# Jisu-Linnea-Han/ClimateMachine.jl

Hardware: AMD Instinct MI355X
Metric: DG RHS DOF-updates/sec (higher is better)
Workload: dtype f64; 1 GPU; Held-Suarez dry GCM (BASELINE configs[2]), stacked cubed sphere 6x30x30x8 elements, N=4, LSRK54 explicit, hyperdiffusion (DryBiharmonic, horizontal), Rusanov, fp64; elements=43200, nodes_per_element=125, states=5, parallelism=element partition (Hilbert, whole columns), 1 rank(s), RCCL p2p halo

## Files before the change

### climatemachine.jl_amd/csrc/cmdg.hip

```cpp
#include <dlfcn.h>

#include <algorithm>
#include <new>
#include <tuple>

#include "rccl.h"
#include "stepping.h"

namespace cmdg {

namespace {
typedef int (*roctx_push_t)(const char *);
typedef int (*roctx_pop_t)();
roctx_push_t g_roctx_push = nullptr;
roctx_pop_t g_roctx_pop = nullptr;
int g_roctx_state = 0;
void roctx_resolve()
{
    g_roctx_state = -1;
    const char *names[] = {"librocprofiler-sdk-roctx.so.1", "librocprofiler-sdk-roctx.so", "libroctx64.so.4",
                           "libroctx64.so", nullptr};
    const char *want = getenv("CMDG_ROCTX");
    void *lib = nullptr;
    for (int i = 0; names[i] && !lib; ++i) lib = dlopen(names[i], RTLD_NOW | RTLD_NOLOAD);
// ... 114 lines not shown
    delete worker;
    worker = nullptr;
    if (s_comp) hipStreamSynchronize(s_comp);
    if (s_comm) hipStreamSynchronize(s_comm);
    prof_collect();
    if (graph_exec) hipGraphExecDestroy(graph_exec);
    if (nccl_comm && rccl::CommDestroy) rccl::CommDestroy(nccl_comm);
}

static __global__ void k_face_digest(const double *__restrict__ vgeo, int nvgeo,
                                     const double *__restrict__ sgeo,
                                     const int64_t *__restrict__ vmapM,
                                     const int64_t *__restrict__ vmapP,
                                     const int64_t *__restrict__ elemtobndy, int NQ, int NQV,
                                     int64_t nreal, int32_t *__restrict__ faceP,
                                     double *__restrict__ faceG, int *__restrict__ bad)
{
    const int Np = NQ * NQ * NQV, Nfph = NQ * NQV, Nfpv = NQ * NQ;
    const int Nfp = Nfph > Nfpv ? Nfph : Nfpv, NFT = 4 * Nfph + 2 * Nfpv;
    const int64_t I = (int64_t)blockIdx.x * blockDim.x + threadIdx.x;
    if (I >= nreal * NFT) return;
    const int64_t e = I / NFT;
    const int t = (int)(I % NFT);
    int f, n;
    if (t < 4 * Nfph) {
        f = t / Nfph;
        n = t % Nfph;
    } else {
        f = 4 + (t - 4 * Nfph) / Nfpv;
        n = (t - 4 * Nfph) % Nfpv;
    }
// ... 3 lines not shown
    switch (f) {
    case 0: vid = NQ * (a + NQ * b); break;
    case 1: vid = (NQ - 1) + NQ * (a + NQ * b); break;
    case 2: vid = a + NQ * NQ * b; break;
    case 3: vid = a + NQ * ((NQ - 1) + NQ * b); break;
    case 4: vid = n; break;
    default: vid = n + NQ * NQ * (NQV - 1); break;
    }
    int flags = 0;
    const int64_t idM = vmapM[o] - 1;
    if (idM != e * Np + vid) flags |= 1;
    int64_t idP = vmapP[o] - 1;
    if (elemtobndy[f + 6 * e] != 0) idP = e * Np + vid;
    if (idP < 0 || idP > 2147483647LL) flags |= 4;
    faceP[I] = (int32_t)idP;
    const double *sg = sgeo + 5 * o;
#pragma unroll
    for (int c = 0; c < 4; ++c) faceG[((int64_t)4 * e + c) * NFT + t] = sg[c];
    const double mi = vgeo[vid + (int64_t)Np * (VMI + (int64_t)nvgeo * e)];
    if (!(sg[SVMI] == mi)) flags |= 2;
    if (flags) atomicOr(bad, flags);
}

int EngineBase::init(const cmdg_desc *d)
{
    Np = NQ * NQ * NQV;
    Nfp = NQ * (NQ > NQV ? NQ : NQV);
    if (d->N[0] != d->N[1] || d->N[0] != NQ - 1 || d->N[2] != NQV - 1)
        return fail(CMDG_ERR_INVALID, "cmdg_create: polynomial orders do not match the engine");
    if (NQV != NQ && !d->Dv)
        return fail(CMDG_ERR_INVALID, "cmdg_create: Dv is required when the vertical order differs");
    nreal = d->nreal;
    nghost = d->nghost;
    nelem = nreal + nghost;
    nf_first = d->nf_first;
// ... 54 lines not shown
    HIPCHK(hipMemcpy(d_D, d->D, sizeof(double) * NQ * NQ, hipMemcpyHostToDevice));
    g.D = d_D;
    g.Dv = d_D;
    if (NQV != NQ) {
        HIPCHK(d_Dv.alloc(NQV * NQV));
        HIPCHK(hipMemcpy(d_Dv, d->Dv, sizeof(double) * NQV * NQV, hipMemcpyHostToDevice));
        g.Dv = d_Dv;
    }
    {
        const int NFT = 4 * NQ * NQV + 2 * NQ * NQ;
        const int64_t nt = std::max<int64_t>(nreal, 1) * NFT;
        DevBuf<int> d_bad;
        int bad = 0;
        HIPCHK(d_faceP.alloc(nt));
        HIPCHK(d_faceG.alloc(4 * nt));
        HIPCHK(d_bad.alloc_zeroed(1, s_comp));
        if (nreal > 0)
            hipLaunchKernelGGL(k_face_digest, dim3((unsigned)((nreal * NFT + 255) / 256)), dim3(256), 0,
                               s_comp, g.vgeo, g.nvgeo, g.sgeo, g.vmapM, g.vmapP, g.elemtobndy, NQ,
                               NQV, nreal, d_faceP.get(), d_faceG.get(), d_bad.get());
        hipError_t le = hipGetLastError();
        hipError_t ce = hipMemcpyAsync(&bad, d_bad, sizeof(int), hipMemcpyDeviceToHost, s_comp);
        hipError_t se = hipStreamSynchronize(s_comp);
        d_bad.reset();
        if (le != hipSuccess || ce != hipSuccess || se != hipSuccess)
            return fail(CMDG_ERR_HIP, "cmdg_create: digest of the face tables failed");
        if (bad & 1)
            return fail(CMDG_ERR_INVALID, "cmdg_create: vmapM is not the face numbering of Grids.jl:586-594");
        if (bad & 2)
            return fail(CMDG_ERR_INVALID, "cmdg_create: sgeo's vMI differs from vgeo's MI at the face nodes (Grids.jl:1097-1101)");
        if (bad & 4)
            return fail(CMDG_ERR_INVALID, "cmdg_create: too many elements for 32-bit face indices");
        g.faceP = d_faceP;
        g.faceG = d_faceG;
    }
    aux = d->state_auxiliary;
    const size_t nd = (size_t)Np * nelem;
    gf = gf_node_major() ? nullptr : d->state_gradient_flux;
    gf_user = gf_node_major() ? d->state_gradient_flux : nullptr;
    if (!gf) {
        HIPCHK(gf_own.alloc_zeroed(std::max<size_t>(nd * ngf, 1), s_comp));
        gf = gf_own;
    }
    hypgrad_user = ngl > 0 ? d->Qhypervisc_grad : nullptr;
    HIPCHK(hypgrad.alloc_zeroed(std::max<size_t>(nd * 3 * ngl, 1), s_comp));
    hypdiv = d->Qhypervisc_div;
    if (!hypdiv) {
        HIPCHK(hd_own.alloc_zeroed(std::max<size_t>(nd * nhyp, 1), s_comp));
        hypdiv = hd_own;
// ... 23 lines not shown
{
    for (int i = 0; i < 2; ++i)
        if (!W[i]) {
            const size_t n = (size_t)Np * ns * nelem;
            HIPCHK(W[i].alloc_zeroed(n, s_comp));
            HIPCHK(hipStreamSynchronize(s_comp));
        }
    return CMDG_OK;
}

int EngineBase::ensure_garg()
{
    if (!garg) {
        const size_t n = std::max<size_t>((size_t)Np * ngl * nelem, 1);
        HIPCHK(garg.alloc_zeroed(n, s_comp));
        HIPCHK(hipStreamSynchronize(s_comp));
    }
    return CMDG_OK;
}

int EngineBase::synchronize()
{
    HIPCHK(hipStreamSynchronize(s_comp));
    HIPCHK(hipStreamSynchronize(s_comm));
    return CMDG_OK;
}

ProfRec &EngineBase::prof_pair(int kernel, bool clamp, Event e1)
{
    ProfRec r{kernel, Event(), std::move(e1), clamp};
// ... 663 lines not shown
```

### climatemachine.jl_amd/csrc/cmdg_common.h

```cpp
#pragma once
#include <hip/hip_runtime.h>
#include <stdint.h>

namespace cmdg {

enum { XI1X1 = 0, XI2X1, XI3X1, XI1X2, XI2X2, XI3X2, XI1X3, XI2X3, XI3X3, VM, VMI };
constexpr int JCV = 15;
enum { SN1 = 0, SN2, SN3, SSM, SVMI };
enum { DIR_EVERY = 0, DIR_HORIZONTAL = 1, DIR_VERTICAL = 2 };
enum {
    NF_RUSANOV = 0, NF_CENTRAL = 1, NF_ROE = 2, NF_HLLC = 3, NF_LMARS = 4,
    NF_ROE_MOIST = 5, NF_ROE_MOIST_LM = 6, NF_ROE_MOIST_HH = 7, NF_ROE_MOIST_LV = 8,
    NF_ROE_MOIST_LVPP = 9
};
enum { BS_FIRST = 0, BS_GRADIENT = 1 };

constexpr int NXCD = 8;

struct GridDev {
    const double *vgeo, *sgeo;
    const int64_t *vmapM, *vmapP, *elemtobndy;
    const double *D;
    const double *Dv;
    int nvgeo;
    const int32_t *faceP;
    const double *faceG;
};

struct SendEnt {
    int32_t node;
    int32_t pos;
};
struct HaloDev {
    const int32_t *sendoff;
    const SendEnt *sendent;
    double *send[2];
    const int32_t *ghostslot;
    const double *recvQ, *recvGF, *recvHG, *recvHD;
    int64_t nreal;
};

// ... 9 lines not shown
    __device__ __forceinline__ static void face_task(int t, int &f, int &n)
    {
        if constexpr (NQ == NQV) {
            f = t / Nfp;
            n = t % Nfp;
        } else if (t < 4 * Nfph) {
            f = t / Nfph;
            n = t % Nfph;
        } else {
            f = 4 + (t - 4 * Nfph) / Nfpv;
            n = (t - 4 * Nfph) % Nfpv;
        }
    }
};

__device__ __forceinline__ int64_t xcd_remap(int64_t b, int64_t G)
{
    const int64_t q = G / NXCD, r = G % NXCD;
    const int64_t x = b % NXCD, y = b / NXCD;
    return x * q + (x < r ? x : r) + y;
}

template <int N>
__device__ __forceinline__ void fill_negzero(double (&a)[N])
{
#pragma unroll
    for (int i = 0; i < N; ++i) a[i] = -0.0;
}
template <int N>
struct Vec {
// ... 55 lines not shown
    } else {
#pragma unroll
        for (int s = 0; s < NLOAD; ++s) dst[s] = arr[hg_at<NHG, Np>(vidP, s, eP)];
    }
}
template <int NHG, int Np, int NW>
__device__ __forceinline__ void store_node_major(double *__restrict__ arr, int64_t e, int tid, int nthreads,
                                                 const double *src)
{
    double *dst = arr + (int64_t)NHG * Np * e;
    for (int m = tid; m < NHG * Np; m += nthreads) {
        const int n = m / NHG, s = m - n * NHG;
        if (NW == NHG || s < NW) dst[m] = src[s * Np + n];
    }
}
template <int NVAR, int NW, class F>
__device__ __forceinline__ void send_nodes(const HaloDev &h, int which, int64_t e, int tid,
                                           int nthreads, F value)
{
    if (h.sendoff == nullptr || h.send[which] == nullptr) return;
    const int b1 = h.sendoff[e + 1];
    for (int k = h.sendoff[e] + tid; k < b1; k += nthreads) {
        const SendEnt ent = h.sendent[k];
        double *dst = h.send[which] + (int64_t)NVAR * ent.pos;
#pragma unroll
        for (int s = 0; s < NW; ++s) dst[s] = value(s, ent.node);
    }
}

}
// ... 1 lines not shown
```

### climatemachine.jl_amd/csrc/engine.h

```cpp
#pragma once
#include "engine_base.h"
#include "kernels.h"

namespace cmdg {

template <class P, int NQ_, int NQV_ = NQ_>
struct EngineT : EngineBase {
    typename P::Params prm;
    PassArgs<P> make_args(const RhsCtx &c, const int64_t *elems, int64_t n, int dir, bool exterior, double *send0,
                          double *send1) const
    {
        PassArgs<P> a;
        a.prm = prm;
        a.g = g;
        a.elems = elems;
        a.nelems = n;
        a.Q = c.Qin;
        a.aux = aux;
        a.aux_rw = aux;
        a.derived = derived;
        a.gf = gf;
        a.hypgrad = hypgrad;
        a.hypdiv = hypdiv;
        a.tendency = c.tendency;
        a.Qout = c.Qout;
        a.garg = garg;
        a.t = c.t;
        a.tptr = c.tptr;
        a.alpha = c.alpha;
        a.beta = c.beta;
        a.rkb_dt = c.rkb_dt;
        a.rka_next = c.rka_next;
        a.direction = dir;
        a.model_dir = direction;
        a.nf_first = nf_first;
        a.h = halo_dev(exterior, send0, send1);
        return a;
    }
    using Kernel = void (*)(PassArgs<P>);
    static constexpr bool HO = GradArgHandoff<P, NQ_, NQV_>::value;
    static constexpr bool ELIDE = GradArgHandoff<P, NQ_, NQV_>::elide_refresh;
// ... 24 lines not shown
    static Kernel tendency_recv(bool recv)
    {
        return recv ? k_tendency<P, NQ_, NQV_, LSRK, GF, true> : k_tendency<P, NQ_, NQV_, LSRK, GF, false>;
    }
    static Kernel pick_tendency(bool lsrk, bool gf, bool recv, GargOut out)
    {
        if constexpr (HO)
            if (out != GargOut::none) {
                if constexpr (ELIDE)
                    if (out == GargOut::records) return k_tendency<P, NQ_, NQV_, true, false, false, true, false>;
                return k_tendency<P, NQ_, NQV_, true, false, false, true>;
            }
        if (lsrk) return gf ? tendency_recv<true, true>(recv) : tendency_recv<true, false>(recv);
        return gf ? tendency_recv<false, true>(recv) : tendency_recv<false, false>(recv);
    }
    void launch_gradients(const RhsCtx &c, const int64_t *elems, int64_t n, bool exterior, hipStream_t st) override
    {
        in_pass(GRADIENTS, n, exterior, st, [&] {
            const PassArgs<P> args = make_args(c, elems, n, diffusion_direction, exterior,
                                               gf_live() ? slot[SLOT_GF].sendbuf : nullptr,
                                               ngl > 0 ? slot[SLOT_HG].sendbuf : nullptr);
            hipLaunchKernelGGL(pick_gradients(gf_live(), c.garg_in), dim3((unsigned)n), dim3(KDims<NQ_, NQV_>::NT), 0,
                               st, args);
        });
    }
    void launch_divgrad(const RhsCtx &c, const int64_t *elems, int64_t n, bool exterior, hipStream_t st) override
    {
        in_pass(DIVGRAD, n, exterior, st, [&] {
            const PassArgs<P> args = make_args(c, elems, n, diffusion_direction, exterior, slot[SLOT_HD].sendbuf, nullptr);
            hipLaunchKernelGGL((k_divgrad<P, NQ_, NQV_>), dim3((unsigned)n), dim3(KDims<NQ_, NQV_>::NT), 0, st, args);
        });
    }
    void launch_gradlap(const RhsCtx &c, const int64_t *elems, int64_t n, bool exterior, hipStream_t st) override
    {
        in_pass(GRADLAP, n, exterior, st, [&] {
            const PassArgs<P> args = make_args(c, elems, n, diffusion_direction, exterior, slot[SLOT_HG].sendbuf, nullptr);
            hipLaunchKernelGGL((k_gradlap<P, NQ_, NQV_>), dim3((unsigned)n), dim3(KDims<NQ_, NQV_>::NT), 0, st, args);
        });
    }
    void launch_tendency(const RhsCtx &c, const int64_t *elems, int64_t n, bool exterior, hipStream_t st) override
    {
        in_pass(TENDENCY, n, exterior, st, [&] {
            using SH = TendencyShape<P, NQ_, NQV_>;
            PassArgs<P> args = make_args(c, elems, n, direction, exterior, c.lsrk ? slot[SLOT_Q].sendbuf : nullptr, nullptr);
            const bool recv = args.h.ghostslot != nullptr && exterior;
            if (!recv) args.h.ghostslot = nullptr;
            hipLaunchKernelGGL(pick_tendency(c.lsrk, P::needs_gradflux(prm), recv, c.garg_out),
                               dim3((unsigned)SH::blocks(n)), dim3(SH::NT), 0, st, args);
        });
    }
    void launch_update_aux(const RhsCtx &c, int64_t e0, int64_t e1) override
    {
// ... 68 lines not shown
```

### climatemachine.jl_amd/csrc/engine_base.h

```cpp
#pragma once
#include <hip/hip_runtime.h>
#include <stdint.h>

#include <algorithm>
#include <condition_variable>
#include <deque>
#include <functional>
#include <mutex>
#include <optional>
#include <string>
#include <thread>
#include <vector>

#include "../../include/cmdg.h"
#include "cmdg_common.h"
#include "owned.h"

namespace cmdg {

enum { SLOT_Q = 0, SLOT_GF = 1, SLOT_HG = 2, SLOT_HD = 3, NSLOT = 4 };
enum { TRANSPORT_NONE = 0, TRANSPORT_LOCAL = 1, TRANSPORT_RCCL = 2 };

struct HaloSlot {
    DevBuf<double> sendbuf, recvbuf;
// ... 9 lines not shown
struct StepInRun {
    bool first_step, last_step;
};

enum class GargOut { none, records, records_refresh };

struct RhsCtx {
    double *tendency = nullptr;
    double *Qin = nullptr;
    double *Qout = nullptr;
    double t = 0, alpha = 1, beta = 0;
    const double *tptr = nullptr;
    bool lsrk = false;
    bool update_after = false;
    bool garg_in = false;
    GargOut garg_out = GargOut::none;
    double rkb_dt = 0, rka_next = 0;
    bool pre_done = false;
};

struct FilterObj {
    int kind = 0, target = 0, direction = 0;
    int nindices = 0;
    int indices[CMDG_MAX_FILTER_STATES] = {0};
    int aux_ref_rho = 0, aux_ref_rhoe = 0;
    DevBuf<double> d_Fh, d_Fv;
};

void roctx_push(const char *name);
void roctx_pop();
// ... 83 lines not shown
    int64_t nreal = 0, nghost = 0, nelem = 0;
    int ns = 0, naux = 0, ngrad = 0, ngf = 0, ngl = 0, nhyp = 0;
    int nf_first = 0, direction = 0, diffusion_direction = 0, stacked = 0;
    GridDev g{};
    const int64_t *d_interior = nullptr, *d_exterior = nullptr;
    const int64_t *d_interior_user = nullptr, *d_exterior_user = nullptr;
    DevBuf<int64_t> d_interior_tiled, d_exterior_tiled;
    int set_stack_height(int nv);
    int set_stream_priority(int level);
    int stream_priority = 0;
    int64_t ninterior = 0, nexterior = 0;
    const uint8_t *d_activedofs = nullptr;
    DevBuf<double> d_D;
    DevBuf<int32_t> d_faceP;
    DevBuf<double> d_faceG;
    const int64_t *d_vmapsend = nullptr, *d_vmaprecv = nullptr;
    int64_t nvmapsend = 0, nvmaprecv = 0;
    std::vector<int> nabrtorank;
    std::vector<int64_t> nabrsend, nabrrecv;
    double *aux = nullptr, *gf = nullptr, *hypdiv = nullptr;
    DevBuf<double> hypgrad;
    DevBuf<double> derived;
    DevBuf<double> gf_own, hd_own;
    double *hypgrad_user = nullptr, *gf_user = nullptr;
    DevBuf<double> gf_scratch;
    bool node_major(const double *array) const
    {
        return array == hypgrad || (array == gf && gf_node_major());
    }
    int dev = 0;
    Event ev_comp;
    HaloSlot slot[NSLOT];
    int slot_nvar_max = 0;
    DevBuf<double> W[2];
    DevBuf<double> garg;
    bool gradarg_handoff = true;
    bool handoff_used = false;
    int64_t handoff_refreshes = 0;
    virtual bool garg_capable() const = 0;
    virtual bool refresh_elidable() const = 0;
    bool handoff_eligible() const
    {
        return gradarg_handoff && garg_capable() && !gf_live() && ngl > 0 && has_update_aux() &&
               fused_update_aux() && !has_hooks && !step_filter && !tendency_filter && !gradient_filter &&
               !step_graph && nghost == 0 && !communicate();
    }
    int ensure_garg();
    DevBuf<double> d_partial;
    int transport = TRANSPORT_NONE;
    int rank = 0, nranks = 1;
// ... 245 lines not shown
```

### climatemachine.jl_amd/csrc/kernels.h

```cpp
#pragma once
#include <type_traits>

#include "cmdg_common.h"

#ifndef CMDG_TEND_MINW
#define CMDG_TEND_MINW 1
#endif
#ifndef CMDG_TEND_EPB_LARGE
#define CMDG_TEND_EPB_LARGE 2
#endif
#ifndef CMDG_TEND_EPB_SMALL
#define CMDG_TEND_EPB_SMALL 1
#endif
#ifndef CMDG_GRAD_MINW
#define CMDG_GRAD_MINW 4
#endif
#ifndef CMDG_GRAD_BOUND_LARGE
#define CMDG_GRAD_BOUND_LARGE 1024
#endif
#ifndef CMDG_LAP_MINW
#define CMDG_LAP_MINW 1
#endif

namespace cmdg {
// ... 2 lines not shown
struct PassArgs {
    typename P::Params prm;
    GridDev g;
    const int64_t *elems;
    int64_t nelems;
    const double *Q;
    const double *aux;
    double *aux_rw;
    const double *derived;
    double *gf;
    double *hypgrad;
    double *hypdiv;
    double *tendency;
    double *Qout;
    double *garg;
    double t, alpha, beta;
    const double *tptr;
    double rkb_dt, rka_next;
    int direction;
    int model_dir;
    int nf_first;
    HaloDev h;
};

struct FacePt {
    double n[3], sM, vMI;
    int64_t eP;
    int vidM, vidP, bctag;
};

template <int NQ, int NQV = NQ>
__host__ __device__ __forceinline__ constexpr int face_vid(int f, int n)
{
    const int a = n % NQ, b = n / NQ;
    switch (f) {
    case 0: return NQ * (a + NQ * b);
    case 1: return (NQ - 1) + NQ * (a + NQ * b);
    case 2: return a + NQ * NQ * b;
    case 3: return a + NQ * ((NQ - 1) + NQ * b);
    case 4: return n;
    default: return n + NQ * NQ * (NQV - 1);
    }
}

template <int NQ, int NQV = NQ>
__device__ __forceinline__ void face_index(const GridDev &g, int64_t e, int t, int f, int32_t &idP,
                                           int &bctag)
{
    idP = g.faceP[(int64_t)KDims<NQ, NQV>::NFT * e + t];
    bctag = (int)g.elemtobndy[f + 6 * e];
}
template <int NQ, int NQV = NQ>
__device__ __forceinline__ void face_geometry(const GridDev &g, int64_t e, int t, int f, int n,
                                              int32_t idP, int bctag, FacePt &fp)
{
    constexpr int Np = KDims<NQ, NQV>::Np, NFT = KDims<NQ, NQV>::NFT;
    const double *sg = g.faceG + (int64_t)4 * NFT * e + t;
    fp.n[0] = sg[0];
    fp.n[1] = sg[NFT];
    fp.n[2] = sg[2 * NFT];
    fp.sM = sg[3 * NFT];
    fp.vidM = face_vid<NQ, NQV>(f, n);
    fp.vMI = g.vgeo[fp.vidM + (int64_t)Np * (VMI + (int64_t)g.nvgeo * e)];
    fp.bctag = bctag;
    fp.eP = idP / Np;
    fp.vidP = idP - (int)fp.eP * Np;
}
template <int NQ, int NQV = NQ>
__device__ __forceinline__ void face_setup(const GridDev &g, int64_t e, int t, int f, int n,
                                           FacePt &fp)
{
    int32_t idP;
    int bctag;
    face_index<NQ, NQV>(g, e, t, f, idP, bctag);
    face_geometry<NQ, NQV>(g, e, t, f, n, idP, bctag, fp);
}

template <class P, class = void>
struct has_flux_wavespeed : std::false_type {
};
template <class P>
struct has_flux_wavespeed<P, std::void_t<decltype(P::HAS_FLUX_WAVESPEED)>> : std::true_type {
};

template <class P, class = void>
struct gf_node_major : std::false_type {
};
template <class P>
struct gf_node_major<P, std::void_t<decltype(P::GF_NODE_MAJOR)>>
    : std::integral_constant<bool, P::GF_NODE_MAJOR && (P::NGF > 0)> {
// ... 651 lines not shown
            if (vt) law_gradient_flux<P>(a.prm, o2, gv, lQ, laux, a_t, Gn);
#pragma unroll
            for (int s = 0; s < NGF; ++s)
                sA[s * Np + tid] = hz ? (vt ? o1[s] + o2[s] : o1[s]) : o2[s];
        }
    }
    __syncthreads();
    Vec<NACC> corr;
    int vidM = 0, fpair = -1;
    if (tid < KD::NFT) {
        int f, n;
        KD::face_task(tid, f, n);
        const bool on = f < 4 ? hz : vt;
        if (on) {
            FacePt fp;
            face_setup<NQ, NQV>(a.g, e, tid, f, n, fp);
            Vec<NS> QM, QP;
            Vec<NAUX> auxM, auxP;
            Vec<NGRAD> GM, GP;
            if constexpr (!GARG_IN) {
                load_state<NS, Np>(QM, a.Q, fp.vidM, e);
                load_state<NAUX, Np>(auxM, a.aux, fp.vidM, e);
            }
#pragma unroll
            for (int s = 0; s < NGRAD; ++s)
                GM[s] = (GMASK >> s & 1) ? sG[s * Np + fp.vidM] : 0.0;
            GP.negzero();
            Vec<NGF> lgf;
            lgf.negzero();
            Vec<3 * NGRAD> tg, nGM;
            if (fp.bctag == 0) {
// ... 34 lines not shown
#pragma unroll
                for (int s = 0; s < NGRAD; ++s)
#pragma unroll
                    for (int d = 0; d < 3; ++d) tg[d + 3 * s] = fp.n[d] * GP[s];
            }
            if constexpr (NGF > 0) law_gradient_flux<P>(a.prm, lgf, tg, QM, auxM, a_t, GM);
#pragma unroll
            for (int s = 0; s < NGRAD; ++s)
#pragma unroll
                for (int d = 0; d < 3; ++d) nGM[d + 3 * s] = fp.n[d] * GM[s];
#pragma unroll
            for (int s = 0; s < NGL; ++s)
#pragma unroll
                for (int d = 0; d < 3; ++d) {
                    const int q = d + 3 * P::hv_indexmap(s);
                    corr[NGF + 3 * s + d] = fp.vMI * fp.sM * (tg[q] - nGM[q]);
                }
            if constexpr (NGF > 0) {
                Vec<NGF> visc;
                for (int s = 0; s < NGF; ++s) visc[s] = 0;
                law_gradient_flux<P>(a.prm, visc, nGM, QM, auxM, a_t, GM);
#pragma unroll
                for (int s = 0; s < NGF; ++s) corr[s] = fp.vMI * fp.sM * (lgf[s] - visc[s]);
            }
            vidM = fp.vidM;
            fpair = f / 2;
        }
    }
#pragma unroll
    for (int p = 0; p < 3; ++p) {
        if (fpair == p) {
#pragma unroll
            for (int s = 0; s < NACC; ++s) sA[s * Np + vidM] += corr[s];
        }
        __syncthreads();
    }
    if (tid < Np) {
        if constexpr (!gf_node_major<P>::value) {
// ... 1 lines not shown
            for (int s = 0; s < NGF; ++s)
                a.gf[tid + (int64_t)Np * (s + (int64_t)P::NGF * e)] = sA[s * Np + tid];
        }
    }
    if constexpr (gf_node_major<P>::value && NGF > 0)
        store_node_major<P::NGF, Np, NGF>(a.gf, e, tid, (int)blockDim.x, sA);
    if constexpr (NHG > 0)
        store_node_major<NHG, Np, NHG>(a.hypgrad, e, tid, (int)blockDim.x, sA + NGF * Np);
    if constexpr (NGF > 0)
        send_nodes<P::NGF, NGF>(a.h, 0, e, tid, (int)blockDim.x, [&](int s, int n) { return sA[s * Np + n]; });
    if constexpr (NHG > 0)
        send_nodes<NHG, NHG>(a.h, 1, e, tid, (int)blockDim.x,
                             [&](int s, int n) { return sA[(NGF + s) * Np + n]; });
}

template <class P, int NQ, int NQV = NQ>
__global__ void __launch_bounds__((KDims<NQ, NQV>::NT)) k_divgrad(const PassArgs<P> a)
{
    using KD = KDims<NQ, NQV>;
    const double a_t = a.tptr ? *a.tptr : a.t;
    constexpr int Np = KD::Np, NAUX = P::NAUX, NGL = P::NGL, NHG = 3 * NGL,
                  NHYP = P::NHYP, NG = NGL > 0 ? NGL : 1;
    __shared__ double sD[NQ * NQ + (NQV == NQ ? 0 : NQV * NQV)];
    const double *const sDv = sD + (NQV == NQ ? 0 : NQ * NQ);
    __shared__ double sC[3 * NG * Np];
    __shared__ double sA[NG * Np];
    constexpr int NSURF = SurfDims<NQ, NQV>::NSURF;
    __shared__ double sM[(NHG > 0 ? NHG : 1) * NSURF];
    const int tid = threadIdx.x;
    const int64_t e = a.elems[xcd_remap(blockIdx.x, gridDim.x)] - 1;
    if (tid < NQ * NQ) sD[tid] = a.g.D[tid];
// ... 49 lines not shown
                for (int kk = 0; kk < NQV; ++kk)
                    dv -= MI * sDv[kk + NQV * k] * sC[(2 * NG + s) * Np + i + NQ * (j + NQ * kk)];
            }
            sA[s * Np + tid] = hz ? (vt ? dh + dv : dh) : dv;
        }
    }
    __syncthreads();
    Vec<NGL> corr;
    int vidM = 0, fpair = -1;
    if (tid < KD::NFT) {
        int f, n;
        KD::face_task(tid, f, n);
        const bool on = f < 4 ? hz : vt;
        if (on) {
            FacePt fp;
            face_setup<NQ, NQV>(a.g, e, tid, f, n, fp);
            Vec<NHG> gM, gP;
            const int sidx = surf_index<NQ, NQV>(fp.vidM);
#pragma unroll
            for (int q = 0; q < NHG; ++q) gM[q] = sM[q * NSURF + sidx];
            load_plus_hg<NHG, Np, NHG>(gP, a.hypgrad, a.h.recvHG, ghost_slot<Np>(a.h, fp.eP, fp.vidP),
                                    fp.vidP, fp.eP);
            if (fp.bctag != 0) {
                Vec<NAUX> auxM, auxP;
                load_state<NAUX, Np>(auxM, a.aux, fp.vidM, e);
                load_state<NAUX, Np>(auxP, a.aux, fp.vidP, fp.eP);
                P::boundary_state_divergence(a.prm, fp.bctag, gP, auxP, fp.n, gM, auxM, a_t);
            }
            const double nh0 = fp.n[0] / 2, nh1 = fp.n[1] / 2, nh2 = fp.n[2] / 2;
#pragma unroll
            for (int s = 0; s < NGL; ++s) {
                const double ldiv = (gP[3 * s] + gM[3 * s]) * nh0 +
                                    (gP[3 * s + 1] + gM[3 * s + 1]) * nh1 +
                                    (gP[3 * s + 2] + gM[3 * s + 2]) * nh2;
                corr[s] = fp.vMI * fp.sM * ldiv;
            }
            vidM = fp.vidM;
            fpair = f / 2;
        }
    }
#pragma unroll
    for (int p = 0; p < 3; ++p) {
        if (fpair == p) {
#pragma unroll
            for (int s = 0; s < NGL; ++s) sA[s * Np + vidM] += corr[s];
        }
        __syncthreads();
    }
    if (tid < Np) {
#pragma unroll
        for (int s = 0; s < NGL; ++s)
            a.hypdiv[tid + (int64_t)Np * (s + (int64_t)NHYP * e)] = sA[s * Np + tid];
    }
    if constexpr (NGL > 0)
        send_nodes<NGL, NGL>(a.h, 0, e, tid, (int)blockDim.x, [&](int s, int n) { return sA[s * Np + n]; });
}

template <class P, int NQ, int NQV = NQ>
__global__ void __launch_bounds__((KDims<NQ, NQV>::NT), CMDG_LAP_MINW) k_gradlap(const PassArgs<P> a)
{
    using KD = KDims<NQ, NQV>;
    const double a_t = a.tptr ? *a.tptr : a.t;
    constexpr int Np = KD::Np, NS = P::NS, NAUX = P::NAUX, NGL = P::NGL,
                  NHG = 3 * NGL, NHYP = P::NHYP, NG = NGL > 0 ? NGL : 1,
                  NH = NHYP > 0 ? NHYP : 1;
    __shared__ double sD[NQ * NQ + (NQV == NQ ? 0 : NQV * NQV)];
    const double *const sDv = sD + (NQV == NQ ? 0 : NQ * NQ);
    __shared__ double sL[NG * Np];
    __shared__ double sA[NH * Np];
    const int tid = threadIdx.x;
    const int64_t e = a.elems[xcd_remap(blockIdx.x, gridDim.x)] - 1;
    if (tid < NQ * NQ) sD[tid] = a.g.D[tid];
    if constexpr (NQV != NQ) {
        if (tid < NQV * NQV) sD[NQ * NQ + tid] = a.g.Dv[tid];
    }
    const bool hz = a.direction != DIR_VERTICAL, vt = a.direction != DIR_HORIZONTAL;
    if (tid < Np) {
        Vec<NGL> l;
#pragma unroll
        for (int s = 0; s < NGL; ++s) l[s] = a.hypdiv[tid + (int64_t)Np * (s + (int64_t)NHYP * e)];
#pragma unroll
        for (int s = 0; s < NGL; ++s) sL[s * Np + tid] = l[s];
    }
    __syncthreads();
    if (tid < Np) {
        const int i = tid % NQ, j = (tid / NQ) % NQ, k = tid / (NQ * NQ);
        const double *vg = a.g.vgeo + (int64_t)Np * a.g.nvgeo * e + tid;
        Vec<NS> lQ;
        Vec<NAUX> laux;
        load_state<NS, Np>(lQ, a.Q, tid, e);
        load_state<NAUX, Np>(laux, a.aux, tid, e);
        Vec<NHG> lh, lv;
        lh.negzero();
        lv.negzero();
        if (hz) {
// ... 33 lines not shown
        h2.negzero();
        if (hz) P::post_gradient_laplacian(a.prm, h1, lh, lQ, laux, a_t);
        if (vt) P::post_gradient_laplacian(a.prm, h2, lv, lQ, laux, a_t);
#pragma unroll
        for (int s = 0; s < NHYP; ++s) sA[s * Np + tid] = hz ? (vt ? h1[s] + h2[s] : h1[s]) : h2[s];
    }
    __syncthreads();
    Vec<NHYP> corr;
    int vidM = 0, fpair = -1;
    if (tid < KD::NFT) {
        int f, n;
        KD::face_task(tid, f, n);
        const bool on = f < 4 ? hz : vt;
        if (on) {
            FacePt fp;
            face_setup<NQ, NQV>(a.g, e, tid, f, n, fp);
            Vec<NS> QM, QP;
            Vec<NAUX> auxM, auxP;
            Vec<NGL> lapM, lapP;
            load_state<NS, Np>(QM, a.Q, fp.vidM, e);
            load_state<NAUX, Np>(auxM, a.aux, fp.vidM, e);
            const int gslot = ghost_slot<Np>(a.h, fp.eP, fp.vidP);
            load_plus<NS, Np, NS>(QP, a.Q, a.h.recvQ, gslot, fp.vidP, fp.eP);
            load_state<NAUX, Np>(auxP, a.aux, fp.vidP, fp.eP);
#pragma unroll
            for (int s = 0; s < NGL; ++s) lapM[s] = sL[s * Np + fp.vidM];
            load_plus<NHYP, Np, NGL, NGL>(lapP, a.hypdiv, a.h.recvHD, gslot, fp.vidP, fp.eP);
            if (fp.bctag != 0)
                P::boundary_state_higher_order(a.prm, fp.bctag, QP, auxP, lapP, fp.n, QM, auxM,
                                               lapM, a_t);
            Vec<NHG> G;
#pragma unroll
            for (int s = 0; s < NGL; ++s)
#pragma unroll
                for (int d = 0; d < 3; ++d) G[d + 3 * s] = fp.n[d] * (lapP[s] - lapM[s]) / 2;
            Vec<NHYP> lh;
            for (int s = 0; s < NHYP; ++s) lh[s] = 0;
            P::post_gradient_laplacian(a.prm, lh, G, QM, auxM, a_t);
#pragma unroll
            for (int s = 0; s < NHYP; ++s) corr[s] = fp.vMI * fp.sM * lh[s];
            vidM = fp.vidM;
            fpair = f / 2;
        }
    }
#pragma unroll
    for (int p = 0; p < 3; ++p) {
        if (fpair == p) {
#pragma unroll
            for (int s = 0; s < NHYP; ++s) sA[s * Np + vidM] += corr[s];
        }
        __syncthreads();
    }
    if constexpr (NHYP > 0) store_node_major<NHG, Np, NHYP>(a.hypgrad, e, tid, (int)blockDim.x, sA);
    if constexpr (NHYP > 0)
        send_nodes<NHG, NHYP>(a.h, 0, e, tid, (int)blockDim.x, [&](int s, int n) { return sA[s * Np + n]; });
// ... 100 lines not shown
```

### climatemachine.jl_amd/csrc/lsrk_run.hip

```cpp
#include "stepping.h"

namespace cmdg {

static __global__ void k_lsrk_update(double *__restrict__ dQ, double *__restrict__ Q, double rka,
                                     double rkb_dt, int64_t n)
{
    for (int64_t i = blockIdx.x * (int64_t)blockDim.x + threadIdx.x; i < n;
         i += (int64_t)gridDim.x * blockDim.x) {
        Q[i] += rkb_dt * dQ[i];
        dQ[i] *= rka;
    }
}
void lsrk_update(hipStream_t st, double *dQ, double *Q, double rka_next, double rkb_dt, int64_t n)
{
    hipLaunchKernelGGL(k_lsrk_update, dim3(nblocks(n)), dim3(256), 0, st, dQ, Q, rka_next, rkb_dt, n);
}
void lsrk_update(EngineBase *e, double *dQ, double *Q, double rka_next, double rkb_dt)
{
    lsrk_update(e->s_comp, dQ, Q, rka_next, rkb_dt, real_len(e));
}

static void lsrk_stage_buffers(EngineBase *e, double *Q, int s, int nstages, double **in, double **out)
{
    *in = s == 0 ? Q : e->W[(s - 1) % 2];
    *out = s == nstages - 1 && nstages > 1 ? Q : e->W[s % 2];
}

struct StageHandoff {
    bool garg_in;
    GargOut out;
};
static StageHandoff handoff_stage(const StepInRun *run, int s, int nstages, bool refresh_elidable)
{
    if (!run) return {false, GargOut::none};
    const bool in = !(run->first_step && s == 0);
    if (run->last_step && s == nstages - 1) return {in, GargOut::none};
    const bool refresh = !refresh_elidable || nstages == 1 || (run->last_step && s == nstages - 2);
    return {in, refresh ? GargOut::records_refresh : GargOut::records};
}

int EngineBase::lsrk_step(double *Q, double *dQ, double t, double dt, int nstages, const double *rka,
                          const double *rkb, const double *rkc, bool continued, const StepInRun *handoff)
{
    std::vector<EngineBase *> one{this};
    double *Qs[1] = {Q}, *dQs[1] = {dQ};
    if (transport == TRANSPORT_LOCAL && communicate())
        return fail(CMDG_ERR_INVALID, "handles connected locally must be driven by the cmdg_group_* calls");
    return group_lsrk_step(one, Qs, dQs, t, dt, nstages, rka, rkb, rkc, continued, nullptr, handoff);
}

int group_lsrk_step(std::vector<EngineBase *> &g, double **Q, double **dQ, double t, double dt,
                    int nstages, const double *rka, const double *rkb, const double *rkc,
                    bool continued, const double *stage_times_dev, const StepInRun *handoff)
// ... 12 lines not shown
                x.Qin = Q[i];
                x.Qout = nullptr;
            }
            x.tendency = dQ[i];
            x.t = t + rkc[s] * dt;
            x.tptr = stage_times_dev ? stage_times_dev + s : nullptr;
            x.alpha = 1.0;
            x.beta = 1.0;
            x.lsrk = fused;
            x.update_after = !fused;
            x.rkb_dt = rkb[s] * dt;
            x.rka_next = rka[(s + 1) % nstages];
            const StageHandoff h = handoff_stage(handoff, s, nstages, g[i]->refresh_elidable());
            x.garg_in = h.garg_in;
            x.garg_out = h.out;
            if (h.out == GargOut::records_refresh) g[i]->handoff_refreshes += 1;
        }
        if (int r = group_rhs(g, c, s > 0 || continued)) return r;
    }
    for (size_t i = 0; i < g.size(); ++i) {
        EngineBase *e = g[i];
        if (nstages == 1 && e->fused_lsrk())
            if (hipMemcpyAsync(Q[i], e->W[0], sizeof(double) * e->Np * e->ns * e->nreal,
                               hipMemcpyDeviceToDevice, e->s_comp) != hipSuccess)
                return e->fail(CMDG_ERR_HIP, "lsrk: copy back failed");
        if (e->step_filter) {
            if (int r = e->filter_apply(e->step_filter, Q[i], e->ns)) return r;
            e->invalidate_sends();
        }
    }
// ... 195 lines not shown
```

Before: 19.11 billion DOF-updates/s.

## Store Laplacian in ring-major records and precompute face lift weights

Face digest now precomputes a per-face-point lift weight (vMI*sM) and a ring-slot-remapped neighbour index. In the handoff path, divgrad writes its Laplacian output to a new ring-major buffer and skips the hypdiv store except on the final evaluation. gradlap then reads neighbour Laplacian values from that buffer via the remapped index and skips loading the plus-side state and aux, reusing the minus side instead. This cuts scattered global loads and extra geometry fetches in the hyperdiffusion face loops, at the cost of two more face tables and another Laplacian buffer. It also assumes the plus-side state and aux are not needed in this path, which holds only if the boundary and flux laws never use them.

```diff
diff --git a/climatemachine.jl_amd/csrc/cmdg.hip b/climatemachine.jl_amd/csrc/cmdg.hip
--- a/climatemachine.jl_amd/csrc/cmdg.hip
+++ b/climatemachine.jl_amd/csrc/cmdg.hip
@@ -152,7 +152,8 @@
                                      const int64_t *__restrict__ vmapP,
                                      const int64_t *__restrict__ elemtobndy, int NQ, int NQV,
                                      int64_t nreal, int32_t *__restrict__ faceP,
-                                     double *__restrict__ faceG, int *__restrict__ bad)
+                                     double *__restrict__ faceG, double *__restrict__ faceW,
+                                     int32_t *__restrict__ facePr, int *__restrict__ bad)
 {
     const int Np = NQ * NQ * NQV, Nfph = NQ * NQV, Nfpv = NQ * NQ;
     const int Nfp = Nfph > Nfpv ? Nfph : Nfpv, NFT = 4 * Nfph + 2 * Nfpv;
@@ -186,11 +187,14 @@
     if (elemtobndy[f + 6 * e] != 0) idP = e * Np + vid;
     if (idP < 0 || idP > 2147483647LL) flags |= 4;
     faceP[I] = (int32_t)idP;
+    const int64_t eP = idP >= 0 ? idP / Np : 0;
+    facePr[I] = (int32_t)(eP * Np + ring_slot_of(NQ, NQV, (int)(idP - eP * Np)));
     const double *sg = sgeo + 5 * o;
 #pragma unroll
     for (int c = 0; c < 4; ++c) faceG[((int64_t)4 * e + c) * NFT + t] = sg[c];
     const double mi = vgeo[vid + (int64_t)Np * (VMI + (int64_t)nvgeo * e)];
     if (!(sg[SVMI] == mi)) flags |= 2;
+    faceW[I] = mi * sg[SSM];
     if (flags) atomicOr(bad, flags);
 }
 
@@ -275,11 +279,14 @@
         int bad = 0;
         HIPCHK(d_faceP.alloc(nt));
         HIPCHK(d_faceG.alloc(4 * nt));
+        HIPCHK(d_faceW.alloc(nt));
+        HIPCHK(d_facePr.alloc(nt));
         HIPCHK(d_bad.alloc_zeroed(1, s_comp));
         if (nreal > 0)
             hipLaunchKernelGGL(k_face_digest, dim3((unsigned)((nreal * NFT + 255) / 256)), dim3(256), 0,
                                s_comp, g.vgeo, g.nvgeo, g.sgeo, g.vmapM, g.vmapP, g.elemtobndy, NQ,
-                               NQV, nreal, d_faceP.get(), d_faceG.get(), d_bad.get());
+                               NQV, nreal, d_faceP.get(), d_faceG.get(), d_faceW.get(), d_facePr.get(),
+                               d_bad.get());
         hipError_t le = hipGetLastError();
         hipError_t ce = hipMemcpyAsync(&bad, d_bad, sizeof(int), hipMemcpyDeviceToHost, s_comp);
         hipError_t se = hipStreamSynchronize(s_comp);
@@ -294,6 +301,8 @@
             return fail(CMDG_ERR_INVALID, "cmdg_create: too many elements for 32-bit face indices");
         g.faceP = d_faceP;
         g.faceG = d_faceG;
+        g.faceW = d_faceW;
+        g.facePr = d_facePr;
     }
     aux = d->state_auxiliary;
     const size_t nd = (size_t)Np * nelem;
@@ -347,6 +356,7 @@
     if (!garg) {
         const size_t n = std::max<size_t>((size_t)Np * ngl * nelem, 1);
         HIPCHK(garg.alloc_zeroed(n, s_comp));
+        HIPCHK(lapr.alloc_zeroed(n, s_comp));
         HIPCHK(hipStreamSynchronize(s_comp));
     }
     return CMDG_OK;
diff --git a/climatemachine.jl_amd/csrc/cmdg_common.h b/climatemachine.jl_amd/csrc/cmdg_common.h
--- a/climatemachine.jl_amd/csrc/cmdg_common.h
+++ b/climatemachine.jl_amd/csrc/cmdg_common.h
@@ -25,6 +25,8 @@
     int nvgeo;
     const int32_t *faceP;
     const double *faceG;
+    const double *faceW;
+    const int32_t *facePr;
 };
 
 struct SendEnt {
@@ -64,6 +66,68 @@
     }
 };
 
+__host__ __device__ __forceinline__ constexpr int ring_slot_of(int NQ, int NQV, int n)
+{
+    const int i = n % NQ, j = (n / NQ) % NQ, k = n / (NQ * NQ), E = NQ - 1;
+    const int c = j == 0 ? i
+                  : i == E ? E + j
+                  : j == E ? 2 * E + (E - i)
+                  : i == 0 ? 3 * E + (E - j)
+                           : 4 * E + (i - 1) + (NQ - 2) * (j - 1);
+    return c * NQV + k;
+}
+__host__ __device__ __forceinline__ constexpr int ring_node_of(int NQ, int NQV, int slot)
+{
+    const int c = slot / NQV, k = slot - c * NQV, E = NQ - 1, NI = NQ > 2 ? NQ - 2 : 1;
+    const int q = c - 4 * E;
+    const int i = c <= E ? c : c <= 2 * E ? E : c <= 3 * E ? 3 * E - c : c < 4 * E ? 0 : 1 + q % NI;
+    const int j = c <= E ? 0 : c <= 2 * E ? c - E : c <= 3 * E ? E : c < 4 * E ? 4 * E - c : 1 + q / NI;
+    return i + NQ * (j + NQ * k);
+}
+template <int NQ, int NQV = NQ>
+__host__ __device__ __forceinline__ constexpr int ring_slot(int n)
+{
+    return ring_slot_of(NQ, NQV, n);
+}
+template <int NQ, int NQV = NQ>
+__host__ __device__ __forceinline__ constexpr int ring_node(int slot)
+{
+    return ring_node_of(NQ, NQV, slot);
+}
+template <int NQ, int NQV>
+constexpr bool ring_order_ok()
+{
+    constexpr int Np = NQ * NQ * NQV, R = 4 * (NQ - 1) * NQV, Nfph = NQ * NQV;
+    for (int n = 0; n < Np; ++n) {
+        const int s = ring_slot<NQ, NQV>(n);
+        if (s < 0 || s >= Np || ring_node<NQ, NQV>(s) != n) return false;
+    }
+    for (int s = 0; s < Np; ++s)
+        if (ring_slot<NQ, NQV>(ring_node<NQ, NQV>(s)) != s) return false;
+    for (int f = 0; f < 4; ++f) {
+        bool on[R] = {};
+        int count = 0;
+        for (int n = 0; n < Np; ++n) {
+            const int i = n % NQ, j = (n / NQ) % NQ;
+            if (f == 0 ? i == 0 : f == 1 ? i == NQ - 1 : f == 2 ? j == 0 : j == NQ - 1) {
+                const int s = ring_slot<NQ, NQV>(n);
+                if (s >= R || on[s]) return false;
+                on[s] = true;
+                ++count;
+            }
+        }
+        if (count != Nfph) return false;
+        int starts = 0;
+        for (int s = 0; s < R; ++s)
+            if (on[s] && !on[(s + R - 1) % R]) ++starts;
+        if (starts != 1) return false;
+    }
+    return true;
+}
+static_assert(ring_order_ok<3, 3>() && ring_order_ok<4, 4>() && ring_order_ok<5, 5>(), "ring order");
+static_assert(ring_order_ok<2, 2>() && ring_order_ok<6, 6>() && ring_order_ok<7, 7>(), "ring order");
+static_assert(ring_order_ok<5, 3>() && ring_order_ok<3, 5>() && ring_order_ok<5, 2>(), "ring order");
+
 __device__ __forceinline__ int64_t xcd_remap(int64_t b, int64_t G)
 {
     const int64_t q = G / NXCD, r = G % NXCD;
@@ -149,6 +213,17 @@
         if (NW == NHG || s < NW) dst[m] = src[s * Np + n];
     }
 }
+template <int NHG, int NQ, int NQV>
+__device__ __forceinline__ void store_ring_major(double *__restrict__ arr, int64_t e, int tid, int nthreads,
+                                                 const double *src)
+{
+    constexpr int Np = KDims<NQ, NQV>::Np;
+    double *dst = arr + (int64_t)NHG * Np * e;
+    for (int m = tid; m < NHG * Np; m += nthreads) {
+        const int r = m / NHG, s = m - r * NHG;
+        dst[m] = src[s * Np + ring_node<NQ, NQV>(r)];
+    }
+}
 template <int NVAR, int NW, class F>
 __device__ __forceinline__ void send_nodes(const HaloDev &h, int which, int64_t e, int tid,
                                            int nthreads, F value)
diff --git a/climatemachine.jl_amd/csrc/engine.h b/climatemachine.jl_amd/csrc/engine.h
--- a/climatemachine.jl_amd/csrc/engine.h
+++ b/climatemachine.jl_amd/csrc/engine.h
@@ -25,6 +25,8 @@
         a.tendency = c.tendency;
         a.Qout = c.Qout;
         a.garg = garg;
+        a.lapr = lapr;
+        a.hypdiv_out = c.hypdiv_out;
         a.t = c.t;
         a.tptr = c.tptr;
         a.alpha = c.alpha;
@@ -79,6 +81,18 @@
         if (lsrk) return gf ? tendency_recv<true, true>(recv) : tendency_recv<true, false>(recv);
         return gf ? tendency_recv<false, true>(recv) : tendency_recv<false, false>(recv);
     }
+    static Kernel pick_divgrad(bool ring)
+    {
+        if constexpr (HO)
+            if (ring) return k_divgrad<P, NQ_, NQV_, true>;
+        return k_divgrad<P, NQ_, NQV_>;
+    }
+    static Kernel pick_gradlap(bool ring)
+    {
+        if constexpr (HO)
+            if (ring) return k_gradlap<P, NQ_, NQV_, true>;
+        return k_gradlap<P, NQ_, NQV_>;
+    }
     void launch_gradients(const RhsCtx &c, const int64_t *elems, int64_t n, bool exterior, hipStream_t st) override
     {
         in_pass(GRADIENTS, n, exterior, st, [&] {
@@ -93,14 +107,15 @@
     {
         in_pass(DIVGRAD, n, exterior, st, [&] {
             const PassArgs<P> args = make_args(c, elems, n, diffusion_direction, exterior, slot[SLOT_HD].sendbuf, nullptr);
-            hipLaunchKernelGGL((k_divgrad<P, NQ_, NQV_>), dim3((unsigned)n), dim3(KDims<NQ_, NQV_>::NT), 0, st, args);
+            hipLaunchKernelGGL(pick_divgrad(c.garg_in), dim3((unsigned)n), dim3(KDims<NQ_, NQV_>::NT), 0, st, args);
         });
     }
     void launch_gradlap(const RhsCtx &c, const int64_t *elems, int64_t n, bool exterior, hipStream_t st) override
     {
         in_pass(GRADLAP, n, exterior, st, [&] {
-            const PassArgs<P> args = make_args(c, elems, n, diffusion_direction, exterior, slot[SLOT_HG].sendbuf, nullptr);
-            hipLaunchKernelGGL((k_gradlap<P, NQ_, NQV_>), dim3((unsigned)n), dim3(KDims<NQ_, NQV_>::NT), 0, st, args);
+            PassArgs<P> args = make_args(c, elems, n, diffusion_direction, exterior, slot[SLOT_HG].sendbuf, nullptr);
+            if (c.garg_in) args.g.faceP = g.facePr;
+            hipLaunchKernelGGL(pick_gradlap(c.garg_in), dim3((unsigned)n), dim3(KDims<NQ_, NQV_>::NT), 0, st, args);
         });
     }
     void launch_tendency(const RhsCtx &c, const int64_t *elems, int64_t n, bool exterior, hipStream_t st) override
diff --git a/climatemachine.jl_amd/csrc/engine_base.h b/climatemachine.jl_amd/csrc/engine_base.h
--- a/climatemachine.jl_amd/csrc/engine_base.h
+++ b/climatemachine.jl_amd/csrc/engine_base.h
@@ -47,6 +47,7 @@
     bool lsrk = false;
     bool update_after = false;
     bool garg_in = false;
+    bool hypdiv_out = true;
     GargOut garg_out = GargOut::none;
     double rkb_dt = 0, rka_next = 0;
     bool pre_done = false;
@@ -160,6 +161,8 @@
     DevBuf<double> d_D;
     DevBuf<int32_t> d_faceP;
     DevBuf<double> d_faceG;
+    DevBuf<double> d_faceW;
+    DevBuf<int32_t> d_facePr;
     const int64_t *d_vmapsend = nullptr, *d_vmaprecv = nullptr;
     int64_t nvmapsend = 0, nvmaprecv = 0;
     std::vector<int> nabrtorank;
@@ -180,6 +183,7 @@
     int slot_nvar_max = 0;
     DevBuf<double> W[2];
     DevBuf<double> garg;
+    DevBuf<double> lapr;
     bool gradarg_handoff = true;
     bool handoff_used = false;
     int64_t handoff_refreshes = 0;
diff --git a/climatemachine.jl_amd/csrc/kernels.h b/climatemachine.jl_amd/csrc/kernels.h
--- a/climatemachine.jl_amd/csrc/kernels.h
+++ b/climatemachine.jl_amd/csrc/kernels.h
@@ -40,6 +40,8 @@
     double *tendency;
     double *Qout;
     double *garg;
+    double *lapr;
+    int hypdiv_out;
     double t, alpha, beta;
     const double *tptr;
     double rkb_dt, rka_next;
@@ -51,6 +53,7 @@
 
 struct FacePt {
     double n[3], sM, vMI;
+    double w;
     int64_t eP;
     int vidM, vidP, bctag;
 };
@@ -76,7 +79,7 @@
     idP = g.faceP[(int64_t)KDims<NQ, NQV>::NFT * e + t];
     bctag = (int)g.elemtobndy[f + 6 * e];
 }
-template <int NQ, int NQV = NQ>
+template <int NQ, int NQV = NQ, bool LIFTW = false>
 __device__ __forceinline__ void face_geometry(const GridDev &g, int64_t e, int t, int f, int n,
                                               int32_t idP, int bctag, FacePt &fp)
 {
@@ -85,21 +88,25 @@
     fp.n[0] = sg[0];
     fp.n[1] = sg[NFT];
     fp.n[2] = sg[2 * NFT];
-    fp.sM = sg[3 * NFT];
     fp.vidM = face_vid<NQ, NQV>(f, n);
-    fp.vMI = g.vgeo[fp.vidM + (int64_t)Np * (VMI + (int64_t)g.nvgeo * e)];
+    if constexpr (LIFTW) {
+        fp.w = g.faceW[(int64_t)NFT * e + t];
+    } else {
+        fp.sM = sg[3 * NFT];
+        fp.vMI = g.vgeo[fp.vidM + (int64_t)Np * (VMI + (int64_t)g.nvgeo * e)];
+    }
     fp.bctag = bctag;
     fp.eP = idP / Np;
     fp.vidP = idP - (int)fp.eP * Np;
 }
-template <int NQ, int NQV = NQ>
+template <int NQ, int NQV = NQ, bool LIFTW = false>
 __device__ __forceinline__ void face_setup(const GridDev &g, int64_t e, int t, int f, int n,
                                            FacePt &fp)
 {
     int32_t idP;
     int bctag;
     face_index<NQ, NQV>(g, e, t, f, idP, bctag);
-    face_geometry<NQ, NQV>(g, e, t, f, n, idP, bctag, fp);
+    face_geometry<NQ, NQV, LIFTW>(g, e, t, f, n, idP, bctag, fp);
 }
 
 template <class P, class = void>
@@ -781,7 +788,7 @@
         const bool on = f < 4 ? hz : vt;
         if (on) {
             FacePt fp;
-            face_setup<NQ, NQV>(a.g, e, tid, f, n, fp);
+            face_setup<NQ, NQV, true>(a.g, e, tid, f, n, fp);
             Vec<NS> QM, QP;
             Vec<NAUX> auxM, auxP;
             Vec<NGRAD> GM, GP;
@@ -846,14 +853,14 @@
 #pragma unroll
                 for (int d = 0; d < 3; ++d) {
                     const int q = d + 3 * P::hv_indexmap(s);
-                    corr[NGF + 3 * s + d] = fp.vMI * fp.sM * (tg[q] - nGM[q]);
+                    corr[NGF + 3 * s + d] = fp.w * (tg[q] - nGM[q]);
                 }
             if constexpr (NGF > 0) {
                 Vec<NGF> visc;
                 for (int s = 0; s < NGF; ++s) visc[s] = 0;
                 law_gradient_flux<P>(a.prm, visc, nGM, QM, auxM, a_t, GM);
 #pragma unroll
-                for (int s = 0; s < NGF; ++s) corr[s] = fp.vMI * fp.sM * (lgf[s] - visc[s]);
+                for (int s = 0; s < NGF; ++s) corr[s] = fp.w * (lgf[s] - visc[s]);
             }
             vidM = fp.vidM;
             fpair = f / 2;
@@ -885,7 +892,7 @@
                              [&](int s, int n) { return sA[(NGF + s) * Np + n]; });
 }
 
-template <class P, int NQ, int NQV = NQ>
+template <class P, int NQ, int NQV = NQ, bool RING = false>
 __global__ void __launch_bounds__((KDims<NQ, NQV>::NT)) k_divgrad(const PassArgs<P> a)
 {
     using KD = KDims<NQ, NQV>;
@@ -965,7 +972,7 @@
         const bool on = f < 4 ? hz : vt;
         if (on) {
             FacePt fp;
-            face_setup<NQ, NQV>(a.g, e, tid, f, n, fp);
+            face_setup<NQ, NQV, true>(a.g, e, tid, f, n, fp);
             Vec<NHG> gM, gP;
             const int sidx = surf_index<NQ, NQV>(fp.vidM);
 #pragma unroll
@@ -984,7 +991,7 @@
                 const double ldiv = (gP[3 * s] + gM[3 * s]) * nh0 +
                                     (gP[3 * s + 1] + gM[3 * s + 1]) * nh1 +
                                     (gP[3 * s + 2] + gM[3 * s + 2]) * nh2;
-                corr[s] = fp.vMI * fp.sM * ldiv;
+                corr[s] = fp.w * ldiv;
             }
             vidM = fp.vidM;
             fpair = f / 2;
@@ -998,16 +1005,19 @@
         }
         __syncthreads();
     }
+    if constexpr (RING) store_ring_major<NG, NQ, NQV>(a.lapr, e, tid, (int)blockDim.x, sA);
     if (tid < Np) {
-#pragma unroll
-        for (int s = 0; s < NGL; ++s)
-            a.hypdiv[tid + (int64_t)Np * (s + (int64_t)NHYP * e)] = sA[s * Np + tid];
+        if (!RING || a.hypdiv_out) {
+#pragma unroll
+            for (int s = 0; s < NGL; ++s)
+                a.hypdiv[tid + (int64_t)Np * (s + (int64_t)NHYP * e)] = sA[s * Np + tid];
+        }
     }
     if constexpr (NGL > 0)
         send_nodes<NGL, NGL>(a.h, 0, e, tid, (int)blockDim.x, [&](int s, int n) { return sA[s * Np + n]; });
 }
 
-template <class P, int NQ, int NQV = NQ>
+template <class P, int NQ, int NQV = NQ, bool RING = false>
 __global__ void __launch_bounds__((KDims<NQ, NQV>::NT), CMDG_LAP_MINW) k_gradlap(const PassArgs<P> a)
 {
     using KD = KDims<NQ, NQV>;
@@ -1028,8 +1038,14 @@
     const bool hz = a.direction != DIR_VERTICAL, vt = a.direction != DIR_HORIZONTAL;
     if (tid < Np) {
         Vec<NGL> l;
-#pragma unroll
-        for (int s = 0; s < NGL; ++s) l[s] = a.hypdiv[tid + (int64_t)Np * (s + (int64_t)NHYP * e)];
+        if constexpr (RING) {
+            const double *rec = a.lapr + garg_at<NG, Np>(ring_slot<NQ, NQV>(tid), e);
+#pragma unroll
+            for (int s = 0; s < NGL; ++s) l[s] = rec[s];
+        } else {
+#pragma unroll
+            for (int s = 0; s < NGL; ++s) l[s] = a.hypdiv[tid + (int64_t)Np * (s + (int64_t)NHYP * e)];
+        }
 #pragma unroll
         for (int s = 0; s < NGL; ++s) sL[s * Np + tid] = l[s];
     }
@@ -1093,18 +1109,30 @@
         const bool on = f < 4 ? hz : vt;
         if (on) {
             FacePt fp;
-            face_setup<NQ, NQV>(a.g, e, tid, f, n, fp);
+            face_setup<NQ, NQV, true>(a.g, e, tid, f, n, fp);
             Vec<NS> QM, QP;
             Vec<NAUX> auxM, auxP;
             Vec<NGL> lapM, lapP;
             load_state<NS, Np>(QM, a.Q, fp.vidM, e);
             load_state<NAUX, Np>(auxM, a.aux, fp.vidM, e);
-            const int gslot = ghost_slot<Np>(a.h, fp.eP, fp.vidP);
-            load_plus<NS, Np, NS>(QP, a.Q, a.h.recvQ, gslot, fp.vidP, fp.eP);
-            load_state<NAUX, Np>(auxP, a.aux, fp.vidP, fp.eP);
-#pragma unroll
-            for (int s = 0; s < NGL; ++s) lapM[s] = sL[s * Np + fp.vidM];
-            load_plus<NHYP, Np, NGL, NGL>(lapP, a.hypdiv, a.h.recvHD, gslot, fp.vidP, fp.eP);
+            if constexpr (RING) {
+#pragma unroll
+                for (int s = 0; s < NS; ++s) QP[s] = QM[s];
+#pragma unroll
+                for (int s = 0; s < NAUX; ++s) auxP[s] = auxM[s];
+#pragma unroll
+                for (int s = 0; s < NGL; ++s) lapM[s] = sL[s * Np + fp.vidM];
+                const double *rec = a.lapr + garg_at<NG, Np>(fp.vidP, fp.eP);
+#pragma unroll
+                for (int s = 0; s < NGL; ++s) lapP[s] = rec[s];
+            } else {
+                const int gslot = ghost_slot<Np>(a.h, fp.eP, fp.vidP);
+                load_plus<NS, Np, NS>(QP, a.Q, a.h.recvQ, gslot, fp.vidP, fp.eP);
+                load_state<NAUX, Np>(auxP, a.aux, fp.vidP, fp.eP);
+#pragma unroll
+                for (int s = 0; s < NGL; ++s) lapM[s] = sL[s * Np + fp.vidM];
+                load_plus<NHYP, Np, NGL, NGL>(lapP, a.hypdiv, a.h.recvHD, gslot, fp.vidP, fp.eP);
+            }
             if (fp.bctag != 0)
                 P::boundary_state_higher_order(a.prm, fp.bctag, QP, auxP, lapP, fp.n, QM, auxM,
                                                lapM, a_t);
@@ -1117,7 +1145,7 @@
             for (int s = 0; s < NHYP; ++s) lh[s] = 0;
             P::post_gradient_laplacian(a.prm, lh, G, QM, auxM, a_t);
 #pragma unroll
-            for (int s = 0; s < NHYP; ++s) corr[s] = fp.vMI * fp.sM * lh[s];
+            for (int s = 0; s < NHYP; ++s) corr[s] = fp.w * lh[s];
             vidM = fp.vidM;
             fpair = f / 2;
         }
diff --git a/climatemachine.jl_amd/csrc/lsrk_run.hip b/climatemachine.jl_amd/csrc/lsrk_run.hip
--- a/climatemachine.jl_amd/csrc/lsrk_run.hip
+++ b/climatemachine.jl_amd/csrc/lsrk_run.hip
@@ -29,14 +29,15 @@
 struct StageHandoff {
     bool garg_in;
     GargOut out;
+    bool last_eval;
 };
 static StageHandoff handoff_stage(const StepInRun *run, int s, int nstages, bool refresh_elidable)
 {
-    if (!run) return {false, GargOut::none};
+    if (!run) return {false, GargOut::none, true};
     const bool in = !(run->first_step && s == 0);
-    if (run->last_step && s == nstages - 1) return {in, GargOut::none};
+    if (run->last_step && s == nstages - 1) return {in, GargOut::none, true};
     const bool refresh = !refresh_elidable || nstages == 1 || (run->last_step && s == nstages - 2);
-    return {in, refresh ? GargOut::records_refresh : GargOut::records};
+    return {in, refresh ? GargOut::records_refresh : GargOut::records, false};
 }
 
 int EngineBase::lsrk_step(double *Q, double *dQ, double t, double dt, int nstages, const double *rka,
@@ -79,6 +80,7 @@
             const StageHandoff h = handoff_stage(handoff, s, nstages, g[i]->refresh_elidable());
             x.garg_in = h.garg_in;
             x.garg_out = h.out;
+            x.hypdiv_out = !h.garg_in || h.last_eval;
             if (h.out == GargOut::records_refresh) g[i]->handoff_refreshes += 1;
         }
         if (int r = group_rhs(g, c, s > 0 || continued)) return r;
```

After: 19.45 billion DOF-updates/s (median of 6 runs). +1.8%, better.
